# crockwell/far

Hardware: AMD Instinct MI355X
Metric: image-pairs/sec (match+solve+regress) at 640x480 (higher is better)
Workload: dtype f32

## Files before the change

far_amd/csrc/emm_bilinear_f16s.hip:

```cpp
#include "common.h"
#include <type_traits>

typedef float f32x4v __attribute__((ext_vector_type(4)));

namespace {

typedef _Float16 f16x8 __attribute__((ext_vector_type(8)));
typedef __attribute__((address_space(1))) const void* gptr_t;
typedef __attribute__((address_space(3))) void* lptr_t;

constexpr int D = 64;
constexpr int DV = 70;
constexpr int DVP = 96;
constexpr int KT = 64;
constexpr int CREF_ROW = 80;
constexpr float QK_PRESCALE = 16.0f;
constexpr float V_PRESCALE = 64.0f;
constexpr float NEG_HUGE = -1.0e30f;
constexpr int PAD_REF = 1 << 24;
constexpr int ROW_REF0 = -(1 << 24);

struct ZLayout {
    int heads, P, rot;
    long head_stride, prob_stride;
    __device__ __forceinline__ size_t base(long z) const {
        const long pz = z / heads;
        const int hh = (int)(z - pz * heads);
        return (size_t)hh * head_stride + (size_t)((pz + rot) % P) * prob_stride;
    }
};

__device__ __forceinline__ void split1(float x, _Float16& hi, _Float16& lo) {
    hi = (_Float16)x;
    lo = (_Float16)(x - (float)hi);
}

__global__ void k_prep_qk(const float* __restrict__ x, ZLayout lay, int Z, int N, int Np, _Float16* __restrict__ hi, _Float16* __restrict__ lo,
                          int* __restrict__ overflow) {
    const long total = (long)Z * Np * 8;
    bool bad = false;
    for (long t = (long)blockIdx.x * blockDim.x + threadIdx.x; t < total; t += (long)gridDim.x * blockDim.x) {
        const int slot = (int)(t & 7);
        const long row = t >> 3;
        const int i = (int)(row % Np);
        const long z = row / Np;
        f16x8 vh, vl;
        if (i < N) {
            const float* src = x + lay.base(z) + (size_t)i * D + slot * 8;
            const float4 a = *reinterpret_cast<const float4*>(src);
            const float4 b = *reinterpret_cast<const float4*>(src + 4);
            const float v[8] = {a.x, a.y, a.z, a.w, b.x, b.y, b.z, b.w};
#pragma unroll
            for (int e = 0; e < 8; ++e) {
                _Float16 h, l;
                split1(v[e] * QK_PRESCALE, h, l);
                vh[e] = h; vl[e] = l;
                bad |= !(fabsf(v[e]) <= 65504.0f / QK_PRESCALE);
            }
        } else {
#pragma unroll
            for (int e = 0; e < 8; ++e) { vh[e] = (_Float16)0.f; vl[e] = (_Float16)0.f; }
        }
        const int s2 = slot ^ ((i >> 1) & 7);
        *reinterpret_cast<f16x8*>(hi + (size_t)row * D + s2 * 8) = vh;
        *reinterpret_cast<f16x8*>(lo + (size_t)row * D + s2 * 8) = vl;
    }
    if (overflow && __any(bad) && (threadIdx.x & 63) == 0) atomicOr(overflow, 1);
}

struct RowFrags {
    f16x8 hi[4], lo[4];
    __device__ __forceinline__ void load(const _Float16* ph, const _Float16* pl, size_t row, int irow, int h) {
#pragma unroll
        for (int s = 0; s < 4; ++s) {
            const int slot = (2 * s + h) ^ ((irow >> 1) & 7);
            hi[s] = *reinterpret_cast<const f16x8*>(ph + row * D + 8 * slot);
            lo[s] = *reinterpret_cast<const f16x8*>(pl + row * D + 8 * slot);
        }
    }
    __device__ __forceinline__ void arrived() {
        asm volatile("s_waitcnt vmcnt(0)" : "+v"(hi[0]), "+v"(hi[1]), "+v"(hi[2]), "+v"(hi[3]),
                                            "+v"(lo[0]), "+v"(lo[1]), "+v"(lo[2]), "+v"(lo[3]) : : "memory");
    }
};

constexpr int CT_PLANE = KT * 128;
__device__ __forceinline__ void dma_col_tile(unsigned char* lds, const _Float16* gh, const _Float16* gl, size_t row0, int tid, int wave) {
    const unsigned char* sh = reinterpret_cast<const unsigned char*>(gh + row0 * D) + tid * 16;
    const unsigned char* sl = reinterpret_cast<const unsigned char*>(gl + row0 * D) + tid * 16;
#pragma unroll
    for (int j = 0; j < 2; ++j) {
        __builtin_amdgcn_global_load_lds((gptr_t)(sh + j * 4096), (lptr_t)(lds + j * 4096 + wave * 1024), 16, 0, 0);
        __builtin_amdgcn_global_load_lds((gptr_t)(sl + j * 4096), (lptr_t)(lds + CT_PLANE + j * 4096 + wave * 1024), 16, 0, 0);
    }
}

__device__ __forceinline__ void glds16(const void* gsrc, unsigned lds_dst_uniform) {
    unsigned keep;
    asm volatile("s_mov_b32 %0, m0\n\ts_mov_b32 m0, %2\n\ts_nop 0\n\tglobal_load_lds_dwordx4 %1, off\n\ts_mov_b32 m0, %0"
                 : "=&s"(keep) : "v"(gsrc), "s"(lds_dst_uniform) : "memory");
}
__device__ __forceinline__ unsigned lds_addr_uniform(const unsigned char* p) {
    return (unsigned)__builtin_amdgcn_readfirstlane((int)(unsigned)(size_t)(lptr_t)p);
}
__device__ __forceinline__ void dma_col_tile_async(unsigned char* lds, const _Float16* gh, const _Float16* gl, size_t row0, int tid, int wave) {
    const unsigned char* sh = reinterpret_cast<const unsigned char*>(gh + row0 * D) + tid * 16;
    const unsigned char* sl = reinterpret_cast<const unsigned char*>(gl + row0 * D) + tid * 16;
    const unsigned dst = lds_addr_uniform(lds + wave * 1024);
#pragma unroll
    for (int j = 0; j < 2; ++j) {
        glds16(sh + j * 4096, dst + j * 4096);
        glds16(sl + j * 4096, dst + CT_PLANE + j * 4096);
    }
}

template <bool SPLIT = true>
__device__ __forceinline__ void score_tile(f32x16 (&acc)[2], const unsigned char* lds, const RowFrags& rf, int l31, int h) {
#pragma unroll
    for (int ct = 0; ct < 2; ++ct)
#pragma unroll
        for (int r = 0; r < 16; ++r) acc[ct][r] = 0.f;
#pragma unroll
    for (int s = 0; s < 4; ++s) {
        f16x8 ch[2], cl[2];
#pragma unroll
        for (int ct = 0; ct < 2; ++ct) {
            const int row = 32 * ct + l31;
            const int off = row * 128 + (((2 * s + h) ^ ((row >> 1) & 7)) * 16);
            ch[ct] = *reinterpret_cast<const f16x8*>(lds + off);
            if (SPLIT) cl[ct] = *reinterpret_cast<const f16x8*>(lds + CT_PLANE + off);
        }
#pragma unroll
        for (int ct = 0; ct < 2; ++ct) acc[ct] = __builtin_amdgcn_mfma_f32_32x32x16_f16(ch[ct], rf.hi[s], acc[ct], 0, 0, 0);
        if (SPLIT) {
#pragma unroll
            for (int ct = 0; ct < 2; ++ct) acc[ct] = __builtin_amdgcn_mfma_f32_32x32x16_f16(ch[ct], rf.lo[s], acc[ct], 0, 0, 0);
#pragma unroll
            for (int ct = 0; ct < 2; ++ct) acc[ct] = __builtin_amdgcn_mfma_f32_32x32x16_f16(cl[ct], rf.hi[s], acc[ct], 0, 0, 0);
        }
    }
}

template <bool MASKED>
__device__ __forceinline__ void rowstat_update(f32x16 (&acc)[2], float c1, int j0, int N, int h, float& m, float& sum, float& comp) {
    float tm = NEG_HUGE;
#pragma unroll
    for (int ct = 0; ct < 2; ++ct)
#pragma unroll
        for (int r = 0; r < 16; ++r) {
            float x = acc[ct][r] * c1;
            if (MASKED && j0 + 32 * ct + mfma32_row(r, h) >= N) x = NEG_HUGE;
            acc[ct][r] = x;
            tm = fmaxf(tm, x);
        }
    const float mn = fmaxf(m, tm);
    const float resc = __builtin_amdgcn_exp2f(m - mn);
    f32x2 t2 = {0.f, 0.f};
    const f32x2 mn2 = {mn, mn};
#pragma unroll
    for (int ct = 0; ct < 2; ++ct)
#pragma unroll
        for (int r = 0; r < 16; r += 2) {
            const f32x2 d = f32x2{acc[ct][r], acc[ct][r + 1]} - mn2;
            t2 += f32x2{__builtin_amdgcn_exp2f(d.x), __builtin_amdgcn_exp2f(d.y)};
        }
    const float t = t2.x + t2.y;
    sum *= resc;
    comp *= resc;
    const float y = t - comp;
    const float ns = sum + y;
    comp = (ns - sum) - y;
    sum = ns;
    m = mn;
}

template <bool SPLIT>
__global__ __launch_bounds__(256, 2) void k_rowstats(const _Float16* __restrict__ ah, const _Float16* __restrict__ al,
                                                     const _Float16* __restrict__ bh, const _Float16* __restrict__ bl,
                                                     int Z, int N, int Np, float c1, float2* __restrict__ stat) {
    __shared__ __attribute__((aligned(16))) unsigned char lds_all[2 * 2 * CT_PLANE];
    const int tid = threadIdx.x, wave = tid >> 6, lane = tid & 63, l31 = lane & 31, h = lane >> 5;
    int z, Ib;
    tile_coords(Np / 128, Z, z, Ib);
    const int irow = Ib * 128 + 32 * wave + l31;
    RowFrags rf;
    rf.load(ah, al, (size_t)z * Np + irow, irow, h);
    rf.arrived();
    float m = NEG_HUGE, sum = 0.f, comp = 0.f;
    const int ntile = Np / KT;
    auto request = [&](int jt) { dma_col_tile_async(lds_all + (jt & 1) * (2 * CT_PLANE), bh, bl, (size_t)z * Np + jt * KT, tid, wave); };
    request(0);
    if (ntile > 1) request(1);
    asm volatile("s_waitcnt vmcnt(0)" ::: "memory");
    __syncthreads();
    f32x16 cur[2];
    score_tile<SPLIT>(cur, lds_all, rf, l31, h);
    for (int jt = 0; jt + 1 < ntile; ++jt) {
        asm volatile("s_waitcnt vmcnt(0)" ::: "memory");
        __syncthreads();
        if (jt + 2 < ntile) request(jt + 2);
        const unsigned char* lds = lds_all + ((jt + 1) & 1) * (2 * CT_PLANE);
        f32x16 nxt[2];
        if ((jt + 1) * KT <= N) {
            score_tile<SPLIT>(nxt, lds, rf, l31, h);
            rowstat_update<false>(cur, c1, jt * KT, N, h, m, sum, comp);
#pragma unroll
            for (int i = 0; i < (SPLIT ? 24 : 0); ++i) {
                if (i < 16) __builtin_amdgcn_sched_group_barrier(0x100, 1, 0);
                __builtin_amdgcn_sched_group_barrier(0x008, 1, 0);
                __builtin_amdgcn_sched_group_barrier(0x002, 6, 0);
            }
        } else {
            score_tile<SPLIT>(nxt, lds, rf, l31, h);
            rowstat_update<true>(cur, c1, jt * KT, N, h, m, sum, comp);
        }
#pragma unroll
        for (int ct = 0; ct < 2; ++ct) cur[ct] = nxt[ct];
    }
    rowstat_update<true>(cur, c1, (ntile - 1) * KT, N, h, m, sum, comp);
    sum -= comp;
    const float mo = shfl_xor_f(m, 32), so = shfl_xor_f(sum, 32);
    const float mn = fmaxf(m, mo);
    const float st = sum * __builtin_amdgcn_exp2f(m - mn) + so * __builtin_amdgcn_exp2f(mo - mn);
    if (h == 0 && irow < N) stat[(size_t)z * N + irow] = make_float2(mn, st);
}

__global__ __launch_bounds__(256) void k_prep_v(const float* __restrict__ v, ZLayout lay, const float* __restrict__ pos,
                                               const float2* __restrict__ colstat, int Z, int N, int Np,
                                               _Float16* __restrict__ oh, _Float16* __restrict__ ol,
                                               int* __restrict__ cref) {
    __shared__ float tile[KT][DV + 3];
    const int ntile = Np / KT;
    const int z = blockIdx.x / ntile, jt = blockIdx.x - z * ntile;
    const int tid = threadIdx.x;
    for (int i = tid; i < KT * DV; i += 256) {
        const int r = i / DV, c = i - r * DV;
        const int j = jt * KT + r;
        float x = 0.f;
        if (j < N) {
            x = c < D ? v[lay.base(z) + (size_t)j * D + c] : pos[(size_t)j * 6 + (c - D)];
            const float2 cs = colstat[(size_t)z * N + j];
            x = x / (cs.y * __builtin_amdgcn_exp2f(cs.x - ceilf(cs.x))) * V_PRESCALE;
        }
        tile[r][c] = x;
    }
    if (tid < KT) {
        const int j = jt * KT + tid;
        cref[(size_t)z * Np + j] = j < N ? (int)ceilf(fminf(fmaxf(colstat[(size_t)z * N + j].x, -1.0e6f), 1.0e6f)) : PAD_REF;
    }
    __syncthreads();
    const size_t base = ((size_t)z * ntile + jt) * DVP * KT;
    for (int i = tid; i < DVP * 8; i += 256) {
        const int b = i >> 3, slot = i & 7;
        const int ct = slot >> 2, g = slot & 3;
        f16x8 vh, vl;
#pragma unroll
        for (int e = 0; e < 8; ++e) {
            const int key = 32 * ct + 16 * (g >> 1) + 4 * (g & 1) + (e < 4 ? e : e + 4);
            const float x = b < DV ? tile[key][b] : 0.f;
            _Float16 hh, ll;
            split1(x, hh, ll);
            vh[e] = hh; vl[e] = ll;
        }
        const size_t o = base + (size_t)b * KT + ((slot ^ ((b >> 1) & 7)) * 8);
        *reinterpret_cast<f16x8*>(oh + o) = vh;
        *reinterpret_cast<f16x8*>(ol + o) = vl;
    }
    __syncthreads();
    if (tid < KT) reinterpret_cast<int*>(oh + base + (size_t)CREF_ROW * KT)[tid] = cref[(size_t)z * Np + jt * KT + tid];
}

constexpr int VT_PLANE = DVP * 128;
constexpr int PV_STAGE = 2 * CT_PLANE + 2 * VT_PLANE;
template <bool MASKED>
__device__ __forceinline__ float tile_rowmax(const f32x16 (&acc)[2], float c1, int j0, int N, int h) {
    float tm = NEG_HUGE;
#pragma unroll
    for (int ct = 0; ct < 2; ++ct)
#pragma unroll
        for (int r = 0; r < 16; ++r) {
            const bool pad = MASKED && j0 + 32 * ct + mfma32_row(r, h) >= N;
            tm = fmaxf(tm, pad ? NEG_HUGE : acc[ct][r]);
        }
    return tm * c1;
}

template <bool SPLIT>
__global__ __launch_bounds__(256, 2) void k_pv(const _Float16* __restrict__ qh, const _Float16* __restrict__ ql,
                                               const _Float16* __restrict__ kh, const _Float16* __restrict__ kl,
                                               const _Float16* __restrict__ vh, const _Float16* __restrict__ vl,
                                               const int* __restrict__ cref, int Z, int N, int Np, float c1,
                                               float2* __restrict__ rowstat, float* __restrict__ T) {
    extern __shared__ __attribute__((aligned(16))) unsigned char lds_all[];
    const int tid = threadIdx.x, wave = tid >> 6, lane = tid & 63, l31 = lane & 31, h = lane >> 5;
    int z, Ib;
    tile_coords(Np / 128, Z, z, Ib);
    const int i0 = Ib * 128 + 32 * wave;
    const int irow = i0 + l31;
    RowFrags rf;
    rf.load(qh, ql, (size_t)z * Np + irow, irow, h);
    rf.arrived();

    f32x16 tacc[3];
#pragma unroll
    for (int bt = 0; bt < 3; ++bt)
#pragma unroll
        for (int r = 0; r < 16; ++r) tacc[bt][r] = 0.f;
    int R = ROW_REF0;
    float sum = 0.f, comp = 0.f;

    const int ntile = Np / KT;
    const unsigned char* vsrc_h = reinterpret_cast<const unsigned char*>(vh + (size_t)z * ntile * DVP * KT) + tid * 16;
    const unsigned char* vsrc_l = reinterpret_cast<const unsigned char*>(vl + (size_t)z * ntile * DVP * KT) + tid * 16;
    auto request = [&](int jt) {
        unsigned char* const st = lds_all + (jt & 1) * PV_STAGE;
        dma_col_tile_async(st, kh, kl, (size_t)z * Np + jt * KT, tid, wave);
        const unsigned dv = lds_addr_uniform(st + 2 * CT_PLANE + wave * 1024);
#pragma unroll
        for (int j = 0; j < 3; ++j) {
            glds16(vsrc_h + (size_t)jt * VT_PLANE + j * 4096, dv + j * 4096);
            glds16(vsrc_l + (size_t)jt * VT_PLANE + j * 4096, dv + VT_PLANE + j * 4096);
        }
    };
    request(0);
    for (int jt = 0; jt < ntile; ++jt) {
        asm volatile("s_waitcnt vmcnt(0)" ::: "memory");
        __syncthreads();
        if (jt + 1 < ntile) request(jt + 1);
        const unsigned char* const lds = lds_all + (jt & 1) * PV_STAGE;
        const unsigned char* const ldv = lds + 2 * CT_PLANE;
        const int* const lcr = reinterpret_cast<const int*>(ldv + CREF_ROW * 128);

        f32x16 acc[2];
        score_tile<SPLIT>(acc, lds, rf, l31, h);
        const bool ragged = (jt + 1) * KT > N;
        const float tm = ragged ? tile_rowmax<true>(acc, c1, jt * KT, N, h) : tile_rowmax<false>(acc, c1, jt * KT, N, h);
        int Rn = (int)ceilf(fminf(fmaxf(tm, -1.0e6f), 1.0e6f));
        Rn = Rn > R ? Rn : R;
        const int Ro = __shfl_xor(Rn, 32, 64);
        Rn = Rn > Ro ? Rn : Ro;
        if (__any(Rn != R)) {
            int d = R - Rn;
            d = d < -200 ? -200 : d;
            sum = ldexpf(sum, d);
            comp = ldexpf(comp, d);
#pragma unroll
            for (int r = 0; r < 16; ++r) {
                const int dr = __shfl(d, mfma32_row(r, h), 64);
#pragma unroll
                for (int bt = 0; bt < 3; ++bt) tacc[bt][r] = ldexpf(tacc[bt][r], dr);
            }
            R = Rn;
        }
        const float nR = -(float)R;
        f32x2 t2 = {0.f, 0.f};
        auto pv_tile = [&](auto ragged_c) {
        constexpr bool RAGGED = decltype(ragged_c)::value;
#pragma unroll
        for (int ct = 0; ct < 2; ++ct) {
#pragma unroll
            for (int u = 0; u < 2; ++u) {
                f16x8 ph, pl;
                const int4 cA = *reinterpret_cast<const int4*>(lcr + 32 * ct + 16 * u + 4 * h);
                const int4 cB = *reinterpret_cast<const int4*>(lcr + 32 * ct + 16 * u + 8 + 4 * h);
                const int cmv[8] = {cA.x, cA.y, cA.z, cA.w, cB.x, cB.y, cB.z, cB.w};
#pragma unroll
                for (int e = 0; e < 8; e += 2) {
                    const int r = 8 * u + e;
                    const f32x2 x2 = __builtin_elementwise_fma(f32x2{acc[ct][r], acc[ct][r + 1]}, f32x2{c1, c1}, f32x2{nR, nR});
                    float e0 = __builtin_amdgcn_exp2f(x2.x);
                    float e1 = __builtin_amdgcn_exp2f(x2.y);
                    if (RAGGED) {
                        if (jt * KT + 32 * ct + mfma32_row(r, h) >= N) e0 = 0.f;
                        if (jt * KT + 32 * ct + mfma32_row(r + 1, h) >= N) e1 = 0.f;
                    }
                    t2 += f32x2{e0, e1};
                    const f32x2 p2 = f32x2{e0, e1} * f32x2{ldexpf(e0, R - cmv[e] + 15), ldexpf(e1, R - cmv[e + 1] + 15)};
                    f16x2 h2, l2;
                    if (SPLIT) split2(p2, h2, l2);
                    else { h2 = __builtin_convertvector(p2, f16x2); l2 = h2; }
                    ph[e] = h2.x; ph[e + 1] = h2.y;
                    pl[e] = l2.x; pl[e + 1] = l2.y;
                }
                const int slot = 4 * ct + 2 * u + h;
#pragma unroll
                for (int bt = 0; bt < 3; ++bt) {
                    const int b = 32 * bt + l31;
                    const int off = b * 128 + ((slot ^ ((b >> 1) & 7)) * 16);
                    const f16x8 bh = *reinterpret_cast<const f16x8*>(ldv + off);
                    tacc[bt] = __builtin_amdgcn_mfma_f32_32x32x16_f16(ph, bh, tacc[bt], 0, 0, 0);
                    if (SPLIT) {
                        const f16x8 bl = *reinterpret_cast<const f16x8*>(ldv + VT_PLANE + off);
                        tacc[bt] = __builtin_amdgcn_mfma_f32_32x32x16_f16(ph, bl, tacc[bt], 0, 0, 0);
                        tacc[bt] = __builtin_amdgcn_mfma_f32_32x32x16_f16(pl, bh, tacc[bt], 0, 0, 0);
                    }
                }
            }
        }
        };
        if (ragged) pv_tile(std::true_type{});
        else pv_tile(std::false_type{});
        const float y = (t2.x + t2.y) - comp;
        const float ns = sum + y;
        comp = (ns - sum) - y;
        sum = ns;
    }
    sum -= comp;
    const float rsum = sum + shfl_xor_f(sum, 32);
    if (h == 0 && irow < N) rowstat[(size_t)z * N + irow] = make_float2((float)R, rsum);
    const float oscale = (3.0517578125e-05f / V_PRESCALE) / rsum;
#pragma unroll
    for (int bt = 0; bt < 3; ++bt) {
        const int b = 32 * bt + l31;
#pragma unroll
        for (int r = 0; r < 16; ++r) {
            const int rr = mfma32_row(r, h);
            const float sc = __shfl(oscale, rr, 64);
            const int i = i0 + rr;
            if (b < DV && i < N) T[((size_t)z * N + i) * DV + b] = tacc[bt][r] * sc;
        }
    }
}

inline size_t align256(size_t x) { return (x + 255) & ~(size_t)255; }
struct EmmWs {
    _Float16 *qh, *ql, *kh, *kl, *vh, *vl;
    float2 *rowstat, *colstat;
    int* cref;
    size_t bytes;
};
inline EmmWs carve(void* base, int Z, int N) {
    const int Np = (N + 127) / 128 * 128;
    unsigned char* p = (unsigned char*)base;
    size_t o = 0;
    auto take = [&](size_t n) { unsigned char* r = p ? p + o : nullptr; o += align256(n); return r; };
    EmmWs w;
    const size_t qk = (size_t)Z * Np * D * 2, vt = (size_t)Z * (Np / KT) * DVP * KT * 2, st = (size_t)Z * N * 8;
    w.qh = (_Float16*)take(qk); w.ql = (_Float16*)take(qk); w.kh = (_Float16*)take(qk); w.kl = (_Float16*)take(qk);
    w.vh = (_Float16*)take(vt); w.vl = (_Float16*)take(vt);
    w.rowstat = (float2*)take(st); w.colstat = (float2*)take(st);
    w.cref = (int*)take((size_t)Z * Np * 4);
    w.bytes = o;
    return w;
}

}

extern "C" {

size_t far_emm_pv_f16s_workspace_bytes(int Z, int N) {
    if (Z <= 0 || N <= 0) return 0;
    return carve(nullptr, Z, N).bytes;
}

}

template <bool SPLIT>
static int emm_pv_launch(const float* q, const float* k, const float* v, const float* pos, int Z, int N, int Dh, float scale,
                         int heads, long head_stride, long prob_stride, int q_rot, void* ws, float* T_out, int* overflow,
                         hipStream_t stream) {
    far_clear_errors();
    if (!q || !k || !v || !pos || !ws || !T_out || Z <= 0 || N <= 0 || Dh != D || heads < 1 || Z % heads || q_rot < 0 ||
        q_rot >= Z / heads)
        return FAR_EINVAL;
    const ZLayout lay{heads, Z / heads, 0, head_stride, prob_stride};
    const ZLayout layq{heads, Z / heads, q_rot, head_stride, prob_stride};
    const int Np = (N + 127) / 128 * 128;
    const EmmWs w = carve(ws, Z, N);
    const float c1 = scale * 1.44269504088896341f / (QK_PRESCALE * QK_PRESCALE);
    const unsigned gprep = (unsigned)(((long)Z * Np * 8 + 255) / 256 < 65536L * 4 ? ((long)Z * Np * 8 + 255) / 256 : 65536L * 4);
    hipLaunchKernelGGL(k_prep_qk, dim3(gprep), dim3(256), 0, stream, q, layq, Z, N, Np, w.qh, w.ql, overflow);
    hipLaunchKernelGGL(k_prep_qk, dim3(gprep), dim3(256), 0, stream, k, lay, Z, N, Np, w.kh, w.kl, overflow);
    const dim3 grid((unsigned)(Np / 128) * Z);
    const dim3 gstat((unsigned)(Np / 128) * Z);
    hipLaunchKernelGGL(k_rowstats<SPLIT>, gstat, dim3(256), 0, stream, w.kh, w.kl, w.qh, w.ql, Z, N, Np, c1, w.colstat);
    hipLaunchKernelGGL(k_prep_v, dim3((unsigned)(Np / KT) * Z), dim3(256), 0, stream, v, lay, pos, w.colstat, Z, N, Np, w.vh, w.vl, w.cref);
    bool cfg_failed = false;
    FAR_ONCE_PER_DEVICE(cfg_failed = hipFuncSetAttribute((const void*)k_pv<SPLIT>, hipFuncAttributeMaxDynamicSharedMemorySize, 2 * PV_STAGE) != hipSuccess);
    if (cfg_failed) return far_check_launch();
    hipLaunchKernelGGL(k_pv<SPLIT>, grid, dim3(256), 2 * PV_STAGE, stream, w.qh, w.ql, w.kh, w.kl, w.vh, w.vl, w.cref, Z, N, Np, c1,
                       w.rowstat, T_out);
    return far_check_launch();
}

extern "C" {

int far_emm_pv_f16s(const float* q, const float* k, const float* v, const float* pos, int Z, int N, int Dh, float scale,
                    int heads, long head_stride, long prob_stride, int q_rot, void* ws, float* T_out, int* overflow,
                    hipStream_t stream) {
    return emm_pv_launch<true>(q, k, v, pos, Z, N, Dh, scale, heads, head_stride, prob_stride, q_rot, ws, T_out, overflow, stream);
}

int far_emm_pv_f16(const float* q, const float* k, const float* v, const float* pos, int Z, int N, int Dh, float scale,
                   int heads, long head_stride, long prob_stride, int q_rot, void* ws, float* T_out, int* overflow,
                   hipStream_t stream) {
    return emm_pv_launch<false>(q, k, v, pos, Z, N, Dh, scale, heads, head_stride, prob_stride, q_rot, ws, T_out, overflow, stream);
}

int far_emm_pv_f16s_copy_stats(const void* ws, int Z, int N, float* rowstat_out, float* colstat_out, hipStream_t stream) {
    far_clear_errors();
    if (!ws || !rowstat_out || !colstat_out || Z <= 0 || N <= 0) return FAR_EINVAL;
    const EmmWs w = carve(const_cast<void*>(ws), Z, N);
    hipMemcpyAsync(rowstat_out, w.rowstat, (size_t)Z * N * 8, hipMemcpyDeviceToDevice, stream);
    hipMemcpyAsync(colstat_out, w.colstat, (size_t)Z * N * 8, hipMemcpyDeviceToDevice, stream);
    return far_check_launch();
}

}
```

far_amd/csrc/head_linear_f32.hip:

```cpp
#include "common.h"

namespace {

constexpr int RB = 32;
__host__ __device__ constexpr int slice_of(int K) { return K > 2048 ? 256 : 64; }

template <int RBT, int KSLT>
__global__ __launch_bounds__(256) void k_rows_partial(const float* __restrict__ x, long ldx, const float4* __restrict__ wp,
                                                      int B, int K, int N, float* __restrict__ partial) {
    constexpr int KT4 = KSLT >= 128 ? 32 : KSLT / 4;
    __shared__ float4 xs[RBT][KT4];
    const int s = blockIdx.x, n = blockIdx.y * 256 + threadIdx.x;
    const int k0 = s * KSLT;
    float acc[RBT];
#pragma unroll
    for (int b = 0; b < RBT; ++b) acc[b] = 0.f;
    const int K4 = (K + 3) >> 2;
    for (int sub = 0; sub < KSLT / (4 * KT4); ++sub) {
        const int kb = k0 + sub * 4 * KT4;
        __syncthreads();
        for (int i = threadIdx.x; i < RBT * KT4; i += 256) {
            const int b = i / KT4, q = i - b * KT4, k = kb + 4 * q;
            float4 v = make_float4(0.f, 0.f, 0.f, 0.f);
            if (b < B) {
                const float* src = x + (long)b * ldx + k;
                if (k + 3 < K) { v.x = src[0]; v.y = src[1]; v.z = src[2]; v.w = src[3]; }
                else { if (k < K) v.x = src[0]; if (k + 1 < K) v.y = src[1]; if (k + 2 < K) v.z = src[2]; }
            }
            xs[b][q] = v;
        }
        __syncthreads();
        if (n < N) {
#pragma unroll 4
            for (int q = 0; q < KT4; ++q) {
                const int k4 = (kb >> 2) + q;
                if (k4 >= K4) break;
                const float4 w = wp[(size_t)k4 * N + n];
#pragma unroll
                for (int b = 0; b < RBT; ++b) {
                    const float4 v = xs[b][q];
                    acc[b] = __builtin_fmaf(v.x, w.x, acc[b]);
                    acc[b] = __builtin_fmaf(v.y, w.y, acc[b]);
                    acc[b] = __builtin_fmaf(v.z, w.z, acc[b]);
                    acc[b] = __builtin_fmaf(v.w, w.w, acc[b]);
                }
            }
        }
    }
    if (n < N)
        for (int b = 0; b < B && b < RBT; ++b) partial[((size_t)s * B + b) * N + n] = acc[b];
}

__global__ void k_rows_reduce(const float* __restrict__ partial, const float* __restrict__ bias, const float* __restrict__ add,
                              long ld_add, int S, int B, int N, int act, float* __restrict__ y, long ldy) {
    const long i = (long)blockIdx.x * blockDim.x + threadIdx.x;
    if (i >= (long)B * N) return;
    const int b = (int)(i / N), n = (int)(i - (long)b * N);
    float v = 0.f;
    for (int s = 0; s < S; ++s) v += partial[((size_t)s * B + b) * N + n];
    if (bias) v += bias[n];
    if (add) v += add[(long)b * ld_add + n];
    if (act == 1) v = fmaxf(v, 0.f);
    else if (act == 2) v = 1.0f / (1.0f + expf(-v));
    else if (act == 3) v = 0.5f * v * (1.0f + erff(v * 0.70710678118654752f));
    y[(long)b * ldy + n] = v;
}

__global__ void k_rows_pack(const float* __restrict__ w, int N, int K, float4* __restrict__ wp) {
    const int K4 = (K + 3) >> 2;
    const long total = (long)K4 * N;
    for (long i = (long)blockIdx.x * blockDim.x + threadIdx.x; i < total; i += (long)gridDim.x * blockDim.x) {
        const int n = (int)(i % N), k = 4 * (int)(i / N);
        const float* src = w + (size_t)n * K + k;
        float4 v;
        v.x = k < K ? src[0] : 0.f; v.y = k + 1 < K ? src[1] : 0.f; v.z = k + 2 < K ? src[2] : 0.f; v.w = k + 3 < K ? src[3] : 0.f;
        wp[i] = v;
    }
}

constexpr int DV = 70, NSEG = 4, VSTR = 72, TSTR = 72;
__global__ __launch_bounds__(256) void k_emm_contract(const float* __restrict__ v, long v_head_stride, long v_prob_stride, int heads,
                                                      const float* __restrict__ pos, const float* __restrict__ T, int N,
                                                      float* __restrict__ part) {
    __shared__ __attribute__((aligned(16))) float vs[64][VSTR], ts[64][TSTR];
    const int z = blockIdx.x, seg = blockIdx.y, Z = gridDim.x;
    const int pz = z / heads, hh = z - pz * heads;
    const float* vz = v + (size_t)hh * v_head_stride + (size_t)pz * v_prob_stride;
    const float* Tz = T + (size_t)z * N * DV;
    const int ntile = (N + 63) / 64, per = (ntile + NSEG - 1) / NSEG;
    const int t0 = seg * per, t1 = min(ntile, t0 + per);
    const int ai = threadIdx.x / 14, bj = threadIdx.x - 14 * ai;
    const bool live = ai < 18;
    float acc[4][5];
#pragma unroll
    for (int i = 0; i < 4; ++i)
#pragma unroll
        for (int j = 0; j < 5; ++j) acc[i][j] = 0.f;
    for (int t = t0; t < t1; ++t) {
        const int n0 = t * 64;
        __syncthreads();
        for (int i = threadIdx.x; i < 64 * VSTR; i += 256) {
            const int r = i / VSTR, c = i - r * VSTR, n = n0 + r;
            float vv = 0.f, tt = 0.f;
            if (n < N && c < DV) {
                vv = c < 64 ? vz[(size_t)n * 64 + c] : pos[(size_t)n * 6 + (c - 64)];
                tt = Tz[(size_t)n * DV + c];
            }
            vs[r][c] = vv; ts[r][c] = tt;
        }
        __syncthreads();
        if (live) {
#pragma unroll 4
            for (int r = 0; r < 64; ++r) {
                const float4 va = *reinterpret_cast<const float4*>(&vs[r][4 * ai]);
                float tb[5];
#pragma unroll
                for (int j = 0; j < 5; ++j) tb[j] = ts[r][5 * bj + j];
                const float a4[4] = {va.x, va.y, va.z, va.w};
#pragma unroll
                for (int i = 0; i < 4; ++i)
#pragma unroll
                    for (int j = 0; j < 5; ++j) acc[i][j] = __builtin_fmaf(a4[i], tb[j], acc[i][j]);
            }
        }
    }
    if (live)
#pragma unroll
        for (int i = 0; i < 4; ++i) {
            const int a = 4 * ai + i;
            if (a < DV)
#pragma unroll
                for (int j = 0; j < 5; ++j) part[(((size_t)seg * Z + z) * DV + a) * DV + 5 * bj + j] = acc[i][j];
        }
}

__global__ void k_emm_contract_sum(const float* __restrict__ part, long per_seg, float* __restrict__ F) {
    const long i = (long)blockIdx.x * blockDim.x + threadIdx.x;
    if (i >= per_seg) return;
    float v = part[i];
#pragma unroll
    for (int s = 1; s < NSEG; ++s) v += part[(size_t)s * per_seg + i];
    F[i] = v;
}

}

extern "C" {

size_t far_rows_linear_packed_bytes(int N, int K) { return (N > 0 && K > 0) ? (size_t)((K + 3) / 4) * N * 16 : 0; }
size_t far_rows_linear_workspace_bytes(int B, int N, int K) {
    return (B > 0 && N > 0 && K > 0) ? (size_t)((K + slice_of(K) - 1) / slice_of(K)) * (B < RB ? B : RB) * N * 4 : 0;
}

int far_rows_linear_pack_f32(const float* w, int N, int K, void* packed, hipStream_t stream) {
    far_clear_errors();
    if (!w || !packed || N <= 0 || K <= 0) return FAR_EINVAL;
    hipLaunchKernelGGL(k_rows_pack, dim3(1024), dim3(256), 0, stream, w, N, K, (float4*)packed);
    return far_check_launch();
}

int far_rows_linear_f32(const float* x, long ldx, const void* packed, const float* bias, const float* add, long ld_add, int B,
                        int K, int N, int act, float* y, long ldy, void* ws, hipStream_t stream) {
    far_clear_errors();
    if (B == 0) return FAR_OK;
    if (!x || !packed || !y || !ws || B < 0 || K <= 0 || N <= 0 || act < 0 || act > 3 || ldx < K || ldy < N || (add && ld_add < N))
        return FAR_EINVAL;
    const int ksl = slice_of(K), S = (K + ksl - 1) / ksl;
    for (int b0 = 0; b0 < B; b0 += RB) {
        const int nb = B - b0 < RB ? B - b0 : RB;
        const dim3 grid(S, (N + 255) / 256);
        const float* xb = x + (long)b0 * ldx;
#define FAR_ROWS_LAUNCH(RBT, KSLT) hipLaunchKernelGGL((k_rows_partial<RBT, KSLT>), grid, dim3(256), 0, stream, xb, ldx, (const float4*)packed, nb, K, N, (float*)ws)
        if (ksl == 256) { if (nb == 1) FAR_ROWS_LAUNCH(1, 256); else if (nb <= 4) FAR_ROWS_LAUNCH(4, 256); else FAR_ROWS_LAUNCH(32, 256); }
        else { if (nb == 1) FAR_ROWS_LAUNCH(1, 64); else if (nb <= 4) FAR_ROWS_LAUNCH(4, 64); else FAR_ROWS_LAUNCH(32, 64); }
#undef FAR_ROWS_LAUNCH
        hipLaunchKernelGGL(k_rows_reduce, dim3((unsigned)(((long)nb * N + 255) / 256)), dim3(256), 0, stream, (const float*)ws, bias,
                           add ? add + (long)b0 * ld_add : nullptr, ld_add, S, nb, N, act, y + (long)b0 * ldy, ldy);
    }
    return far_check_launch();
}

size_t far_emm_contract_workspace_bytes(int Z) { return Z > 0 ? (size_t)NSEG * Z * DV * DV * 4 : 0; }
int far_emm_contract_f32(const float* v, int heads, long head_stride, long prob_stride, const float* pos, const float* T, int Z,
                         int N, float* F, void* ws, hipStream_t stream) {
    far_clear_errors();
    if (Z == 0) return FAR_OK;
    if (!v || !pos || !T || !F || !ws || Z < 0 || N <= 0 || heads < 1 || Z % heads) return FAR_EINVAL;
    hipLaunchKernelGGL(k_emm_contract, dim3(Z, NSEG), dim3(256), 0, stream, v, head_stride, prob_stride, heads, pos, T, N, (float*)ws);
    const long per_seg = (long)Z * DV * DV;
    hipLaunchKernelGGL(k_emm_contract_sum, dim3((unsigned)((per_seg + 255) / 256)), dim3(256), 0, stream, (const float*)ws, per_seg, F);
    return far_check_launch();
}

}
```

far_amd/flags.py:

```python
import os
from collections import namedtuple

Switch = namedtuple('Switch', 'env module attr off_value neutral scope doc')
SWITCHES = [
    Switch('FAR_NO_WINO', 'far_amd.ops', 'USE_WINO', False, 'parity', 'inference',
           'stride-1 3x3 convolutions on K9 (direct implicit GEMM) instead of K17 (Winograd F(2x2,3x3)); same operator, other summation'),
    Switch('FAR_NO_PAD', 'far_amd.loftr.backbone', 'PAD_CHANNELS', False, 'bitwise', 'inference',
           'the 196-channel backbone maps stored with 196 channels instead of 208 (zero weights for the extra ones: exact zeros)'),
    Switch('FAR_NO_PREFETCH', 'far_amd.loftr.model:LoFTR', 'head_prefetch', False, 'bitwise', 'inference',
           "the head's feature stage computed inside forward_rt_prediction instead of enqueued behind K1"),
    Switch('FAR_NO_SIDE_STREAM', 'far_amd.loftr.model:LoFTR', 'head_side_stream', False, 'bitwise', 'inference',
           "the head's feature stage on the step's own stream behind K1 (rounds 2-5) instead of on a second stream next to K1 and the fine level"),
    Switch('FAR_FPN_STREAM', 'far_amd.loftr.model:LoFTR', 'fpn_side_stream', True, 'bitwise', 'inference',
           "OPT-IN (1 switches it ON; default off): the FPN's fine branch on a side stream next to the coarse transformer and K1 (-0.6 ms per 32 "
           "pairs; off by default because the roofline launch -- K17 208 -> 208 @ 240x320 -- then shares the GPU and its in-step duration "
           "in a kernel trace is no longer its own)"),
    Switch('FAR_NO_GATHER_FUSE', 'far_amd.loftr.stages:FinePreprocess', 'fused_gather', False, 'bitwise', 'inference',
           'FinePreprocess.merge_feat on a materialised window tensor (K3 gather + K9) instead of K9 reading through the match indices'),
    Switch('FAR_NO_KV', 'far_amd.loftr.transformer:LoFTREncoderLayer', 'fused_kv', False, 'parity', 'inference',
           "k, v projections + K5's first half as separate launches instead of K9's k|v epilogue (the K'^T V sum changes order)"),
    Switch('FAR_NO_QAPPLY', 'far_amd.loftr.transformer:LoFTREncoderLayer', 'fused_apply', False, 'parity', 'inference',
           "q projection + K5's second half as separate launches instead of K9's attention-apply epilogue (q no longer stays in split operands)"),
    Switch('FAR_NO_STACK', 'far_amd.loftr.transformer:LocalFeatureTransformer', 'stack_self', False, 'bitwise', 'inference',
           "the two 'self' calls of an encoder layer on the two images separately instead of one call on both"),
    Switch('FAR_NO_BN', 'far_amd.ops', 'USE_HIP_BATCHNORM_TRAIN', False, 'parity', 'training',
           'training-mode BatchNorm on nn.BatchNorm2d + torch activations instead of K19 (tests/test_train_kernels_gpu.py holds K19 to the module)'),
]

ENV_ONLY = {
    'FAR_HIP_LIB': ('load', 'path of another build of libfar_hip.so (tools/ab_build.py: same-box A/B against a git revision); skips the build-id check'),
    'FAR_TUNING': ('load', 'comma-separated key=value pairs handed to far_set_tuning at load time, e.g. FAR_TUNING="10=1,8=1" (keys below)'),
    'FAR_SKIP_ASM_CHECK': ('build', "1: far_amd/build.py does not scan the generated code (K9's asm pixel loads; the LDS-DMA ring rule of every kernel with global_load_lds; the half-register writes of the asm fp16 split) after recompiling"),
    'FAR_EXTRA_HIPCC_FLAGS': ('build', 'extra hipcc flags of an experiment build (-DFAR_WINO_EXP=..., tools/wino_exp.sh); part of the build id'),
    'FAR_COMMIT': ('tools', 'commit stamp tools/collect_profiles.sh / tools/step_floors.py write into the profile files'),
    'FAR_C3_PY_NODE': ('bench', "bench.py --workload c3: the encoder layer's autograd node driven from Python instead of far_enc_layer_fwd / _bwd"),
    'FAR_C3_NO_OVERLAP': ('bench', 'bench.py --workload c3: the layer node without side streams'),
    'FAR_C3_PER_OP': ('bench', 'bench.py --workload c3: one autograd node per operator instead of per layer'),
    'FAR_TORCH_ADAMW': ('bench', 'bench.py --workload c3: torch.optim.AdamW instead of K20'),
    'FAR_CUDNN_BENCHMARK': ('bench', 'bench.py: torch.backends.cudnn.benchmark for the vendor comparison legs'),
}

Tuning = namedtuple('Tuning', 'key default values neutral doc')
TUNING = [
    Tuning(0, 3, (0, 1, 2, 4, 7), 'bitwise', 'bit mask of exact-f32 kernels that stagger wave-slot priorities: 1 k_stats, 2 k_match, 4 k_emm_pv'),
    Tuning(1, 0, (1,), 'parity', 'K1 exact-f32 variant: the other tile shape (another summation order of the row statistics)'),
    Tuning(2, 0, (1,), 'bitwise', 'conf_matrix writer variant A (store pattern)'),
    Tuning(3, 0, (1,), 'bitwise', 'conf_matrix writer variant B (store pattern)'),
    Tuning(4, 0, (1,), 'bitwise', 'K9 without the seven-tile mode / K5 windows on the generic path'),
    Tuning(5, 0, (1, 2, 4), 'bitwise', 'K5 apply: tiles per unit'),
    Tuning(6, 0, (64, 256), 'parity', "K5: tokens per K'^T V chunk (another partial-sum grouping)"),
    Tuning(7, 0, (1,), 'bitwise', 'K9 Linear launches always on full-height tiles'),
    Tuning(8, 0, (1,), 'bitwise', 'K17 splits its operands with the five-instruction split2 instead of v_fma_mix (same values)'),
    Tuning(9, 0, (1,), 'bitwise', 'K17 runs a short last channel block on the full body'),
    Tuning(10, 0, (1,), 'bitwise', "K1's match pass without the tile prescreen"),
    Tuning(11, 0, (1, 2), 'bitwise', "K14's pipeline: 0 = 4 waves / 3 slots / counted waits, two workgroups per CU; 1 = 8 waves / 4 slots / counted, one per CU (round 5's form); 2 = 4 waves / 3 slots / vmcnt(0) per phase (fallback without a wait table)"),
    Tuning(12, 0, (1,), 'parity', "K10's inference form on the exact-f32 matrix instruction instead of split fp16"),
    Tuning(15, 0, (1,), 'bitwise', 'K17: 1 = the multiplying wave group does NOT raise its issue priority (the round-4 kernel)'),
    Tuning(13, 0, (1,), 'bitwise', "K9's FPN-merge epilogue in its generic form everywhere"),
]


def off(env):
    if env not in {s.env for s in SWITCHES}:
        raise KeyError(f'{env} is not a registered far_amd switch (far_amd/flags.py)')
    return os.environ.get(env, '0') not in ('', '0')


def value(env, default=None):
    if env not in ENV_ONLY:
        raise KeyError(f'{env} is not a registered far_amd environment variable (far_amd/flags.py)')
    return os.environ.get(env, default)


def known():
    return {s.env for s in SWITCHES} | set(ENV_ONLY)


def unknown_in_environment():
    skip = ('FAR_WINO_', 'FAR_K9_')
    return sorted(k for k in os.environ if k.startswith('FAR_') and k not in known() and not k.startswith(skip))


def target(sw):
    import importlib
    mod, _, cls = sw.module.partition(':')
    obj = importlib.import_module(mod)
    return (getattr(obj, cls) if cls else obj), sw.attr
```

Measured before the change: 381.1.

## Fuse head operand prep launches, prefetch contract tiles, regroup row-partial GEMV

After: 381.4 (median of 5 runs). Within noise of the previous version (+0.1%).

```diff
diff --git a/far_amd/csrc/emm_bilinear_f16s.hip b/far_amd/csrc/emm_bilinear_f16s.hip
--- a/far_amd/csrc/emm_bilinear_f16s.hip
+++ b/far_amd/csrc/emm_bilinear_f16s.hip
@@ -35,35 +35,51 @@
     lo = (_Float16)(x - (float)hi);
 }
 
+__device__ __forceinline__ void prep_qk_slot(const float* __restrict__ x, const ZLayout& lay, long t, int N, int Np,
+                                             _Float16* __restrict__ hi, _Float16* __restrict__ lo, bool& bad) {
+    const int slot = (int)(t & 7);
+    const long row = t >> 3;
+    const int i = (int)(row % Np);
+    const long z = row / Np;
+    f16x8 vh, vl;
+    if (i < N) {
+        const float* src = x + lay.base(z) + (size_t)i * D + slot * 8;
+        const float4 a = *reinterpret_cast<const float4*>(src);
+        const float4 b = *reinterpret_cast<const float4*>(src + 4);
+        const float v[8] = {a.x, a.y, a.z, a.w, b.x, b.y, b.z, b.w};
+#pragma unroll
+        for (int e = 0; e < 8; ++e) {
+            _Float16 h, l;
+            split1(v[e] * QK_PRESCALE, h, l);
+            vh[e] = h; vl[e] = l;
+            bad |= !(fabsf(v[e]) <= 65504.0f / QK_PRESCALE);
+        }
+    } else {
+#pragma unroll
+        for (int e = 0; e < 8; ++e) { vh[e] = (_Float16)0.f; vl[e] = (_Float16)0.f; }
+    }
+    const int s2 = slot ^ ((i >> 1) & 7);
+    *reinterpret_cast<f16x8*>(hi + (size_t)row * D + s2 * 8) = vh;
+    *reinterpret_cast<f16x8*>(lo + (size_t)row * D + s2 * 8) = vl;
+}
+
 __global__ void k_prep_qk(const float* __restrict__ x, ZLayout lay, int Z, int N, int Np, _Float16* __restrict__ hi, _Float16* __restrict__ lo,
                           int* __restrict__ overflow) {
     const long total = (long)Z * Np * 8;
     bool bad = false;
-    for (long t = (long)blockIdx.x * blockDim.x + threadIdx.x; t < total; t += (long)gridDim.x * blockDim.x) {
-        const int slot = (int)(t & 7);
-        const long row = t >> 3;
-        const int i = (int)(row % Np);
-        const long z = row / Np;
-        f16x8 vh, vl;
-        if (i < N) {
-            const float* src = x + lay.base(z) + (size_t)i * D + slot * 8;
-            const float4 a = *reinterpret_cast<const float4*>(src);
-            const float4 b = *reinterpret_cast<const float4*>(src + 4);
-            const float v[8] = {a.x, a.y, a.z, a.w, b.x, b.y, b.z, b.w};
-#pragma unroll
-            for (int e = 0; e < 8; ++e) {
-                _Float16 h, l;
-                split1(v[e] * QK_PRESCALE, h, l);
-                vh[e] = h; vl[e] = l;
-                bad |= !(fabsf(v[e]) <= 65504.0f / QK_PRESCALE);
-            }
-        } else {
-#pragma unroll
-            for (int e = 0; e < 8; ++e) { vh[e] = (_Float16)0.f; vl[e] = (_Float16)0.f; }
-        }
-        const int s2 = slot ^ ((i >> 1) & 7);
-        *reinterpret_cast<f16x8*>(hi + (size_t)row * D + s2 * 8) = vh;
-        *reinterpret_cast<f16x8*>(lo + (size_t)row * D + s2 * 8) = vl;
+    for (long t = (long)blockIdx.x * blockDim.x + threadIdx.x; t < total; t += (long)gridDim.x * blockDim.x)
+        prep_qk_slot(x, lay, t, N, Np, hi, lo, bad);
+    if (overflow && __any(bad) && (threadIdx.x & 63) == 0) atomicOr(overflow, 1);
+}
+
+__global__ void k_prep_qk2(const float* __restrict__ q, ZLayout layq, const float* __restrict__ k, ZLayout lay, int Z, int N, int Np,
+                           _Float16* __restrict__ qh, _Float16* __restrict__ ql, _Float16* __restrict__ kh, _Float16* __restrict__ kl,
+                           int* __restrict__ overflow) {
+    const long total = (long)Z * Np * 8;
+    bool bad = false;
+    for (long t = (long)blockIdx.x * blockDim.x + threadIdx.x; t < 2 * total; t += (long)gridDim.x * blockDim.x) {
+        if (t < total) prep_qk_slot(q, layq, t, N, Np, qh, ql, bad);
+        else prep_qk_slot(k, lay, t - total, N, Np, kh, kl, bad);
     }
     if (overflow && __any(bad) && (threadIdx.x & 63) == 0) atomicOr(overflow, 1);
 }
@@ -174,10 +190,24 @@
     m = mn;
 }
 
-template <bool SPLIT>
+struct PrepV {
+    const float* v;
+    ZLayout lay;
+    const float* pos;
+    _Float16 *oh, *ol;
+    int* cref;
+};
+typedef int i32x4 __attribute__((ext_vector_type(4)));
+constexpr int VP_TSTR = DV + 3;
+constexpr int VP_STAT = KT * VP_TSTR * 4;
+constexpr int VP_CREF = VP_STAT + 128 * 8;
+static_assert(VP_CREF + 128 * 4 <= 2 * 2 * CT_PLANE && VP_STAT % 16 == 0 && VP_CREF % 16 == 0, "the tail's LDS fits the stage buffers");
+static_assert(((CREF_ROW >> 1) & 7) == 0 && CREF_ROW + 1 < DVP && CREF_ROW >= DV, "reference rows: unswizzled padding rows");
+
+template <bool SPLIT, bool PREPV>
 __global__ __launch_bounds__(256, 2) void k_rowstats(const _Float16* __restrict__ ah, const _Float16* __restrict__ al,
                                                      const _Float16* __restrict__ bh, const _Float16* __restrict__ bl,
-                                                     int Z, int N, int Np, float c1, float2* __restrict__ stat) {
+                                                     int Z, int N, int Np, float c1, float2* __restrict__ stat, PrepV pv) {
     __shared__ __attribute__((aligned(16))) unsigned char lds_all[2 * 2 * CT_PLANE];
     const int tid = threadIdx.x, wave = tid >> 6, lane = tid & 63, l31 = lane & 31, h = lane >> 5;
     int z, Ib;
@@ -223,6 +253,86 @@
     const float mn = fmaxf(m, mo);
     const float st = sum * __builtin_amdgcn_exp2f(m - mn) + so * __builtin_amdgcn_exp2f(mo - mn);
     if (h == 0 && irow < N) stat[(size_t)z * N + irow] = make_float2(mn, st);
+    if constexpr (PREPV) {
+        float4 xv[2][4];
+        float xp[2][2];
+        {
+            const float* const vz = pv.v + pv.lay.base(z);
+#pragma unroll
+            for (int tt = 0; tt < 2; ++tt) {
+#pragma unroll
+                for (int u = 0; u < 4; ++u) {
+                    const int i = tid + 256 * u, j = (2 * Ib + tt) * KT + (i >> 4);
+                    xv[tt][u] = make_float4(0.f, 0.f, 0.f, 0.f);
+                    if (j < N) xv[tt][u] = *reinterpret_cast<const float4*>(vz + (size_t)j * D + 4 * (i & 15));
+                }
+#pragma unroll
+                for (int u = 0; u < 2; ++u) {
+                    const int i = tid + 256 * u, r = i / (DV - D), j = (2 * Ib + tt) * KT + r;
+                    xp[tt][u] = 0.f;
+                    if (i < KT * (DV - D) && j < N) xp[tt][u] = pv.pos[(size_t)j * 6 + (i - r * (DV - D))];
+                }
+            }
+        }
+        float (*tile)[VP_TSTR] = reinterpret_cast<float (*)[VP_TSTR]>(lds_all);
+        float2* const cs_s = reinterpret_cast<float2*>(lds_all + VP_STAT);
+        int* const cr_s = reinterpret_cast<int*>(lds_all + VP_CREF);
+        ring_barrier();  
+        if (h == 0) {
+            const int cr = irow < N ? (int)ceilf(fminf(fmaxf(mn, -1.0e6f), 1.0e6f)) : PAD_REF;
+            cs_s[32 * wave + l31] = make_float2(mn, st);
+            cr_s[32 * wave + l31] = cr;
+            pv.cref[(size_t)z * Np + irow] = cr;
+        }
+#pragma unroll
+        for (int tt = 0; tt < 2; ++tt) {
+            const int jt = 2 * Ib + tt;
+            ring_barrier();
+#pragma unroll
+            for (int u = 0; u < 4; ++u) {
+                const int i = tid + 256 * u, r = i >> 4, c4 = i & 15;
+                float4 x = xv[tt][u];
+                if (jt * KT + r < N) {
+                    const float2 cs = cs_s[tt * KT + r];
+                    const float den = cs.y * __builtin_amdgcn_exp2f(cs.x - ceilf(cs.x));
+                    x.x = x.x / den * V_PRESCALE; x.y = x.y / den * V_PRESCALE; x.z = x.z / den * V_PRESCALE; x.w = x.w / den * V_PRESCALE;
+                }
+                tile[r][4 * c4] = x.x; tile[r][4 * c4 + 1] = x.y; tile[r][4 * c4 + 2] = x.z; tile[r][4 * c4 + 3] = x.w;
+            }
+#pragma unroll
+            for (int u = 0; u < 2; ++u) {
+                const int i = tid + 256 * u, r = i / (DV - D), c = i - r * (DV - D);
+                if (i < KT * (DV - D)) {
+                    float x = xp[tt][u];
+                    if (jt * KT + r < N) {
+                        const float2 cs = cs_s[tt * KT + r];
+                        x = x / (cs.y * __builtin_amdgcn_exp2f(cs.x - ceilf(cs.x))) * V_PRESCALE;
+                    }
+                    tile[r][D + c] = x;
+                }
+            }
+            ring_barrier();  
+            const size_t base = ((size_t)z * ntile + jt) * DVP * KT;
+            for (int i = tid; i < DVP * 8; i += 256) {
+                const int b = i >> 3, slot = i & 7;
+                const int ct = slot >> 2, g = slot & 3;
+                f16x8 vh, vl;
+#pragma unroll
+                for (int e = 0; e < 8; ++e) {
+                    const int key = 32 * ct + 16 * (g >> 1) + 4 * (g & 1) + (e < 4 ? e : e + 4);
+                    const float x = b < DV ? tile[key][b] : 0.f;
+                    _Float16 hh, ll;
+                    split1(x, hh, ll);
+                    vh[e] = hh; vl[e] = ll;
+                }
+                if (b == CREF_ROW || b == CREF_ROW + 1)
+                    vh = __builtin_bit_cast(f16x8, *reinterpret_cast<const i32x4*>(cr_s + tt * KT + 32 * (b - CREF_ROW) + 4 * slot));
+                const size_t o = base + (size_t)b * KT + ((slot ^ ((b >> 1) & 7)) * 8);
+                *reinterpret_cast<f16x8*>(pv.oh + o) = vh;
+                *reinterpret_cast<f16x8*>(pv.ol + o) = vl;
+            }
+        }
+    }
 }
 
 __global__ __launch_bounds__(256) void k_prep_v(const float* __restrict__ v, ZLayout lay, const float* __restrict__ pos,
@@ -468,13 +578,22 @@
     const int Np = (N + 127) / 128 * 128;
     const EmmWs w = carve(ws, Z, N);
     const float c1 = scale * 1.44269504088896341f / (QK_PRESCALE * QK_PRESCALE);
-    const unsigned gprep = (unsigned)(((long)Z * Np * 8 + 255) / 256 < 65536L * 4 ? ((long)Z * Np * 8 + 255) / 256 : 65536L * 4);
-    hipLaunchKernelGGL(k_prep_qk, dim3(gprep), dim3(256), 0, stream, q, layq, Z, N, Np, w.qh, w.ql, overflow);
-    hipLaunchKernelGGL(k_prep_qk, dim3(gprep), dim3(256), 0, stream, k, lay, Z, N, Np, w.kh, w.kl, overflow);
+    const long nslot = (long)Z * Np * 8;
+    auto blocks = [](long n) { return (unsigned)((n + 255) / 256 < 65536L * 4 ? (n + 255) / 256 : 65536L * 4); };
     const dim3 grid((unsigned)(Np / 128) * Z);
     const dim3 gstat((unsigned)(Np / 128) * Z);
-    hipLaunchKernelGGL(k_rowstats<SPLIT>, gstat, dim3(256), 0, stream, w.kh, w.kl, w.qh, w.ql, Z, N, Np, c1, w.colstat);
-    hipLaunchKernelGGL(k_prep_v, dim3((unsigned)(Np / KT) * Z), dim3(256), 0, stream, v, lay, pos, w.colstat, Z, N, Np, w.vh, w.vl, w.cref);
+    const bool v_aligned = (((size_t)v | (size_t)head_stride * 4 | (size_t)prob_stride * 4) & 15) == 0;
+    if (!(far_get_tuning(14) & 1) && v_aligned) {
+        const PrepV pv{v, lay, pos, w.vh, w.vl, w.cref};
+        hipLaunchKernelGGL(k_prep_qk2, dim3(blocks(2 * nslot)), dim3(256), 0, stream, q, layq, k, lay, Z, N, Np, w.qh, w.ql, w.kh, w.kl, overflow);
+        hipLaunchKernelGGL((k_rowstats<SPLIT, true>), gstat, dim3(256), 0, stream, w.kh, w.kl, w.qh, w.ql, Z, N, Np, c1, w.colstat, pv);
+    } else {
+        const PrepV none{};
+        hipLaunchKernelGGL(k_prep_qk, dim3(blocks(nslot)), dim3(256), 0, stream, q, layq, Z, N, Np, w.qh, w.ql, overflow);
+        hipLaunchKernelGGL(k_prep_qk, dim3(blocks(nslot)), dim3(256), 0, stream, k, lay, Z, N, Np, w.kh, w.kl, overflow);
+        hipLaunchKernelGGL((k_rowstats<SPLIT, false>), gstat, dim3(256), 0, stream, w.kh, w.kl, w.qh, w.ql, Z, N, Np, c1, w.colstat, none);
+        hipLaunchKernelGGL(k_prep_v, dim3((unsigned)(Np / KT) * Z), dim3(256), 0, stream, v, lay, pos, w.colstat, Z, N, Np, w.vh, w.vl, w.cref);
+    }
     bool cfg_failed = false;
     FAR_ONCE_PER_DEVICE(cfg_failed = hipFuncSetAttribute((const void*)k_pv<SPLIT>, hipFuncAttributeMaxDynamicSharedMemorySize, 2 * PV_STAGE) != hipSuccess);
     if (cfg_failed) return far_check_launch();
diff --git a/far_amd/csrc/head_linear_f32.hip b/far_amd/csrc/head_linear_f32.hip
--- a/far_amd/csrc/head_linear_f32.hip
+++ b/far_amd/csrc/head_linear_f32.hip
@@ -49,6 +49,67 @@
     }
     if (n < N)
         for (int b = 0; b < B && b < RBT; ++b) partial[((size_t)s * B + b) * N + n] = acc[b];
+}
+
+constexpr int RG = 8;
+template <int KSLT>
+__global__ __launch_bounds__(256) void k_rows_partial_g8(const float* __restrict__ x, long ldx, const float4* __restrict__ wp,
+                                                         int B, int K, int N, float* __restrict__ partial) {
+    constexpr int KT4 = 32, QG = 8;
+    static_assert(KSLT % (4 * KT4) == 0 && RB == 4 * RG, "whole LDS tiles per slice; four row groups per workgroup");
+    __shared__ float4 xs[RB][KT4];
+    const int s = blockIdx.x, n = blockIdx.y * 64 + (threadIdx.x & 63);
+    const int b0 = (threadIdx.x >> 6) * RG;
+    const int k0 = s * KSLT;
+    const bool work = n < N && b0 < B;
+    float acc[RG];
+#pragma unroll
+    for (int b = 0; b < RG; ++b) acc[b] = 0.f;
+    const int K4 = (K + 3) >> 2;
+    auto quad = [&](const float4 w, int q) {
+#pragma unroll
+        for (int b = 0; b < RG; ++b) {
+            const float4 v = xs[b0 + b][q];
+            acc[b] = __builtin_fmaf(v.x, w.x, acc[b]);
+            acc[b] = __builtin_fmaf(v.y, w.y, acc[b]);
+            acc[b] = __builtin_fmaf(v.z, w.z, acc[b]);
+            acc[b] = __builtin_fmaf(v.w, w.w, acc[b]);
+        }
+    };
+    for (int sub = 0; sub < KSLT / (4 * KT4); ++sub) {
+        const int kb = k0 + sub * 4 * KT4;
+        __syncthreads();
+        for (int i = threadIdx.x; i < RB * KT4; i += 256) {
+            const int b = i / KT4, q = i - b * KT4, k = kb + 4 * q;
+            float4 v = make_float4(0.f, 0.f, 0.f, 0.f);
+            if (b < B) {
+                const float* src = x + (long)b * ldx + k;
+                if (k + 3 < K) { v.x = src[0]; v.y = src[1]; v.z = src[2]; v.w = src[3]; }
+                else { if (k < K) v.x = src[0]; if (k + 1 < K) v.y = src[1]; if (k + 2 < K) v.z = src[2]; }
+            }
+            xs[b][q] = v;
+        }
+        __syncthreads();
+        if (work) {
+            const int qn = min(KT4, K4 - (kb >> 2));
+            const float4* wq = wp + (size_t)(kb >> 2) * N + n;
+            if (qn == KT4) {
+                for (int q0 = 0; q0 < KT4; q0 += QG) {
+                    float4 w[QG];
+#pragma unroll
+                    for (int u = 0; u < QG; ++u) w[u] = wq[(size_t)(q0 + u) * N];
+#pragma unroll
+                    for (int u = 0; u < QG; ++u) quad(w[u], q0 + u);
+                }
+            } else {
+                for (int q = 0; q < qn; ++q) quad(wq[(size_t)q * N], q);
+            }
+        }
+    }
+    if (work)
+#pragma unroll
+        for (int b = 0; b < RG; ++b)
+            if (b0 + b < B) partial[((size_t)s * B + b0 + b) * N + n] = acc[b];
 }
 
 __global__ void k_rows_reduce(const float* __restrict__ partial, const float* __restrict__ bias, const float* __restrict__ add,
@@ -79,7 +140,7 @@
 }
 
 constexpr int DV = 70, NSEG = 4, VSTR = 72, TSTR = 72;
-__global__ __launch_bounds__(256) void k_emm_contract(const float* __restrict__ v, long v_head_stride, long v_prob_stride, int heads,
+__global__ __launch_bounds__(256) void k_emm_contract_ld1(const float* __restrict__ v, long v_head_stride, long v_prob_stride, int heads,
                                                       const float* __restrict__ pos, const float* __restrict__ T, int N,
                                                       float* __restrict__ part) {
     __shared__ __attribute__((aligned(16))) float vs[64][VSTR], ts[64][TSTR];
@@ -134,6 +195,125 @@
         }
 }
 
+
+template <int W> struct VecOf;
+template <> struct VecOf<4> { typedef float4 type; };
+template <> struct VecOf<2> { typedef float2 type; };
+
+template <int W>
+__device__ __forceinline__ void emm_contract_segment(const float* __restrict__ vz, const float* __restrict__ pos, const float* __restrict__ Tz,
+                                                     int N, int t0, int t1, int ai, int bj, bool live, float (&acc)[4][5],
+                                                     float (*vs)[VSTR], float* ts) {
+    typedef typename VecOf<W>::type VT;
+    constexpr int NT = (64 * DV / W + 255) / 256;
+    const int tid = threadIdx.x;
+    float4 rv[4], rp;
+    VT rt[NT];
+    auto fetch = [&](int t) {
+        const int n0 = t * 64, rows = min(64, N - n0);
+#pragma unroll
+        for (int u = 0; u < 4; ++u) {
+            const int idx = tid + 256 * u, r = idx >> 4, c4 = idx & 15;
+            rv[u] = make_float4(0.f, 0.f, 0.f, 0.f);
+            if (r < rows) rv[u] = *reinterpret_cast<const float4*>(vz + (size_t)(n0 + r) * 64 + 4 * c4);
+        }
+        rp = make_float4(0.f, 0.f, 0.f, 0.f);
+        if (tid < 96) {
+            const float* src = pos + (size_t)n0 * 6;
+            const int e = 4 * tid, lim = rows * 6;
+            if (e + 4 <= lim) rp = *reinterpret_cast<const float4*>(src + e);
+            else { if (e < lim) rp.x = src[e]; if (e + 1 < lim) rp.y = src[e + 1]; if (e + 2 < lim) rp.z = src[e + 2]; }
+        }
+        const float* src = Tz + (size_t)n0 * DV;
+        const int lim = rows * DV;
+#pragma unroll
+        for (int u = 0; u < NT; ++u) {
+            const int e = (tid + 256 * u) * W;
+            VT x;
+            if constexpr (W == 4) {
+                x = make_float4(0.f, 0.f, 0.f, 0.f);
+                if (e + 4 <= lim) x = *reinterpret_cast<const float4*>(src + e);
+                else if (e + 2 <= lim) { const float2 h2 = *reinterpret_cast<const float2*>(src + e); x.x = h2.x; x.y = h2.y; }
+            } else {
+                x = make_float2(0.f, 0.f);
+                if (e + 2 <= lim) x = *reinterpret_cast<const float2*>(src + e);
+            }
+            rt[u] = x;
+        }
+    };
+    auto stash = [&]() {
+#pragma unroll
+        for (int u = 0; u < 4; ++u) {
+            const int idx = tid + 256 * u, r = idx >> 4, c4 = idx & 15;
+            *reinterpret_cast<float4*>(&vs[r][4 * c4]) = rv[u];
+        }
+        if (tid < 96) {
+            const float p4[4] = {rp.x, rp.y, rp.z, rp.w};
+#pragma unroll
+            for (int i = 0; i < 4; ++i) {
+                const int e = 4 * tid + i;
+                vs[e / 6][64 + e % 6] = p4[i];
+            }
+        }
+#pragma unroll
+        for (int u = 0; u < NT; ++u) {
+            const int e = (tid + 256 * u) * W;
+            if (e < 64 * DV) *reinterpret_cast<VT*>(ts + e) = rt[u];
+        }
+    };
+    if (tid < 64) { vs[tid][DV] = 0.f; vs[tid][DV + 1] = 0.f; }
+    if (t0 < t1) fetch(t0);
+    for (int t = t0; t < t1; ++t) {
+        __syncthreads();
+        stash();
+        __syncthreads();
+        if (t + 1 < t1) fetch(t + 1);
+        if (live) {
+#pragma unroll 4
+            for (int r = 0; r < 64; ++r) {
+                const float4 va = *reinterpret_cast<const float4*>(&vs[r][4 * ai]);
+                float tb[5];
+#pragma unroll
+                for (int j = 0; j < 5; ++j) tb[j] = ts[r * DV + 5 * bj + j];
+                const float a4[4] = {va.x, va.y, va.z, va.w};
+#pragma unroll
+                for (int i = 0; i < 4; ++i)
+#pragma unroll
+                    for (int j = 0; j < 5; ++j) acc[i][j] = __builtin_fmaf(a4[i], tb[j], acc[i][j]);
+            }
+        }
+    }
+}
+
+__global__ __launch_bounds__(256) void k_emm_contract(const float* __restrict__ v, long v_head_stride, long v_prob_stride, int heads,
+                                                      const float* __restrict__ pos, const float* __restrict__ T, int N,
+                                                      float* __restrict__ part) {
+    __shared__ __attribute__((aligned(16))) float vs[64][VSTR], ts[64 * DV];
+    const int z = blockIdx.x, seg = blockIdx.y, Z = gridDim.x;
+    const int pz = z / heads, hh = z - pz * heads;
+    const float* vz = v + (size_t)hh * v_head_stride + (size_t)pz * v_prob_stride;
+    const float* Tz = T + (size_t)z * N * DV;
+    const int ntile = (N + 63) / 64, per = (ntile + NSEG - 1) / NSEG;
+    const int t0 = seg * per, t1 = min(ntile, t0 + per);
+    const int ai = threadIdx.x / 14, bj = threadIdx.x - 14 * ai;
+    const bool live = ai < 18;
+    float acc[4][5];
+#pragma unroll
+    for (int i = 0; i < 4; ++i)
+#pragma unroll
+        for (int j = 0; j < 5; ++j) acc[i][j] = 0.f;
+    if ((((size_t)z * N) & 1) == 0) emm_contract_segment<4>(vz, pos, Tz, N, t0, t1, ai, bj, live, acc, vs, ts);
+    else emm_contract_segment<2>(vz, pos, Tz, N, t0, t1, ai, bj, live, acc, vs, ts);
+    if (live)
+#pragma unroll
+        for (int i = 0; i < 4; ++i) {
+            const int a = 4 * ai + i;
+            if (a < DV)
+#pragma unroll
+                for (int j = 0; j < 5; ++j) part[(((size_t)seg * Z + z) * DV + a) * DV + 5 * bj + j] = acc[i][j];
+        }
+}
+
 __global__ void k_emm_contract_sum(const float* __restrict__ part, long per_seg, float* __restrict__ F) {
     const long i = (long)blockIdx.x * blockDim.x + threadIdx.x;
     if (i >= per_seg) return;
@@ -171,7 +351,12 @@
         const dim3 grid(S, (N + 255) / 256);
         const float* xb = x + (long)b0 * ldx;
 #define FAR_ROWS_LAUNCH(RBT, KSLT) hipLaunchKernelGGL((k_rows_partial<RBT, KSLT>), grid, dim3(256), 0, stream, xb, ldx, (const float4*)packed, nb, K, N, (float*)ws)
-        if (ksl == 256) { if (nb == 1) FAR_ROWS_LAUNCH(1, 256); else if (nb <= 4) FAR_ROWS_LAUNCH(4, 256); else FAR_ROWS_LAUNCH(32, 256); }
+        if (ksl == 256) {
+            if (nb == 1) FAR_ROWS_LAUNCH(1, 256);
+            else if (nb <= 4) FAR_ROWS_LAUNCH(4, 256);
+            else if (far_get_tuning(14) & 4) FAR_ROWS_LAUNCH(32, 256);
+            else hipLaunchKernelGGL((k_rows_partial_g8<256>), dim3(S, (N + 63) / 64), dim3(256), 0, stream, xb, ldx, (const float4*)packed, nb, K, N, (float*)ws);
+        }
         else { if (nb == 1) FAR_ROWS_LAUNCH(1, 64); else if (nb <= 4) FAR_ROWS_LAUNCH(4, 64); else FAR_ROWS_LAUNCH(32, 64); }
 #undef FAR_ROWS_LAUNCH
         hipLaunchKernelGGL(k_rows_reduce, dim3((unsigned)(((long)nb * N + 255) / 256)), dim3(256), 0, stream, (const float*)ws, bias,
@@ -186,7 +371,11 @@
     far_clear_errors();
     if (Z == 0) return FAR_OK;
     if (!v || !pos || !T || !F || !ws || Z < 0 || N <= 0 || heads < 1 || Z % heads) return FAR_EINVAL;
-    hipLaunchKernelGGL(k_emm_contract, dim3(Z, NSEG), dim3(256), 0, stream, v, head_stride, prob_stride, heads, pos, T, N, (float*)ws);
+    const bool aligned = (((size_t)v | (size_t)pos | (size_t)T | (size_t)head_stride * 4 | (size_t)prob_stride * 4) & 15) == 0;
+    if (aligned && !(far_get_tuning(14) & 2))
+        hipLaunchKernelGGL(k_emm_contract, dim3(Z, NSEG), dim3(256), 0, stream, v, head_stride, prob_stride, heads, pos, T, N, (float*)ws);
+    else
+        hipLaunchKernelGGL(k_emm_contract_ld1, dim3(Z, NSEG), dim3(256), 0, stream, v, head_stride, prob_stride, heads, pos, T, N, (float*)ws);
     const long per_seg = (long)Z * DV * DV;
     hipLaunchKernelGGL(k_emm_contract_sum, dim3((unsigned)((per_seg + 255) / 256)), dim3(256), 0, stream, (const float*)ws, per_seg, F);
     return far_check_launch();
diff --git a/far_amd/flags.py b/far_amd/flags.py
--- a/far_amd/flags.py
+++ b/far_amd/flags.py
@@ -55,6 +55,7 @@
     Tuning(10, 0, (1,), 'bitwise', "K1's match pass without the tile prescreen"),
     Tuning(11, 0, (1, 2), 'bitwise', "K14's pipeline: 0 = 4 waves / 3 slots / counted waits, two workgroups per CU; 1 = 8 waves / 4 slots / counted, one per CU (round 5's form); 2 = 4 waves / 3 slots / vmcnt(0) per phase (fallback without a wait table)"),
     Tuning(12, 0, (1,), 'parity', "K10's inference form on the exact-f32 matrix instruction instead of split fp16"),
+    Tuning(14, 0, (1, 2, 4, 7), 'bitwise', "bit mask of the head's helper kernels in their previous forms: 1 K2's operand preparation as three launches (k_prep_qk x 2, k_prep_v) instead of k_prep_qk2 + the tail of k_rowstats, 2 k_emm_contract with 4-byte tile loads and no prefetch, 4 K15's 256-k slices on 32 row slots per thread"),
     Tuning(15, 0, (1,), 'bitwise', 'K17: 1 = the multiplying wave group does NOT raise its issue priority (the round-4 kernel)'),
     Tuning(13, 0, (1,), 'bitwise', "K9's FPN-merge epilogue in its generic form everywhere"),
 ]
```
